# vidify/old-audiosync

Measured on AMD Instinct MI355X. Metric: cross-correlations/sec (N=1440000 float32 pairs), higher is better.
Workload: dtype f32

## Files before the change

### include/audiosync/xcorr_hip.h

```cpp
#ifndef AUDIOSYNC_XCORR_HIP_H
#define AUDIOSYNC_XCORR_HIP_H

#include <stddef.h>
#include <stdint.h>

#ifdef __cplusplus
extern "C" {
#endif

typedef struct asx_plan asx_plan;


int asx_device_count(void);
int asx_current_device(void);
const char *asx_last_error(void);
int asx_abi_version(void);


asx_plan *asx_plan_create(size_t sample_len, size_t max_batch, int device);
asx_plan *asx_plan_create_ex(size_t sample_len, size_t max_batch, int device, const char *split);
int asx_plan_placement(asx_plan *plan, double ms[2], int *kept);
void asx_plan_destroy(asx_plan *plan);

int asx_plan_peak_overflows(asx_plan *plan, uint64_t *count);
int asx_plan_peak_repairs(asx_plan *plan, uint64_t *count);
int asx_plan_set_exact(asx_plan *plan, int on);
size_t asx_plan_peak_capacity(const asx_plan *plan);

int asx_plan_set_pearson(asx_plan *plan, int spectral);
int asx_plan_pearson_modes(asx_plan *plan, uint64_t counts[3]);

size_t asx_plan_sample_len(const asx_plan *plan);
size_t asx_plan_fft_len(const asx_plan *plan);
int asx_plan_split(const asx_plan *plan, int *m1, int *m2, int *tile_cols);
int asx_plan_layout(const asx_plan *plan);
int asx_plan_threads(const asx_plan *plan, int *threads_cols, int *threads_rows);
size_t asx_plan_group(const asx_plan *plan);
size_t asx_plan_workspace_bytes(const asx_plan *plan);


int asx_xcorr_f64(asx_plan *plan, const double *source, const double *sample, long *lag,
                  double *coefficient);
int asx_plan_narrowed_calls(asx_plan *plan, uint64_t *count);

int asx_xcorr_batch_f32(asx_plan *plan, const float *source, const float *sample, size_t batch,
// ... 62 lines not shown
```

### old-audiosync_amd/csrc/asx_api.hip

```cpp
#include "audiosync/xcorr_hip.h"

#include "asx_internal.h"
#include "plan_math.h"
#include "shard_driver.h"
#include "host_narrow.h"

#include <algorithm>
#include <cstdarg>
#include <cstdio>
#include <cstdlib>
#include <cstring>
#include <dlfcn.h>
#include <mutex>
#include <string>
#include <thread>
#include <vector>

static thread_local std::string g_err;

static int fail(const char *fmt, ...)
{
    char buf[512];
    va_list ap;
    va_start(ap, fmt);
// ... 73 lines not shown
        AsxCand *cand = nullptr;
        uint32_t *refine_idx = nullptr, *cand_n = nullptr, *refine_n = nullptr;
        double *refine_val = nullptr;
        unsigned long long *overflows = nullptr;
        float *src_dc = nullptr;
        double *stats = nullptr;
        size_t cap = 0;
    } big;
    uint32_t *over_list = nullptr, *over_n = nullptr;
    volatile uint32_t *h_over_n = nullptr;
    size_t over_cap = 0;
    std::vector<uint32_t> h_over;
    unsigned long long repaired = 0;
    bool exact = true;
    bool spectral = false;
    unsigned long long *mode_count = nullptr;
    bool tune_placement = false, placement_done = false;
    double placement_ms[2] = { 0.0, 0.0 };
    int placement_kept = -1;
    float *st_src = nullptr, *st_smp = nullptr;
    int64_t *st_lag = nullptr;
    double *st_coef = nullptr;
    int32_t *st_ret = nullptr;
    double *st_src64 = nullptr, *st_smp64 = nullptr;
    float *pin32 = nullptr;
    unsigned long long narrowed = 0;

    bool profiling = false;
    size_t prof_depth = 1, prof_calls = 0, prof_ring = 0;
    std::vector<std::vector<hipEvent_t>> evr;
// ... 73 lines not shown
    cap = std::min<size_t>(cap, 2 * N);
    for (int l = 0; l < p->nlanes; l++) {
        asx_plan::Lane &ln = p->lanes[l];
        ln.pk.cap = (uint32_t)cap;
        const size_t mz = ((size_t)h.M1 + 1) * (size_t)h.M2;
        if (dev_alloc(p, &ln.zxa, g * mz) || dev_alloc(p, &ln.zya, g * mz) || dev_alloc(p, &ln.ga, g * mz) ||
            dev_alloc(p, &ln.pk.nrm_part, g * 2 * (size_t)h.ntiles) || dev_alloc(p, &ln.pk.bound2, g) ||
            dev_alloc(p, &ln.pk.pairmax, g) || dev_alloc(p, &ln.pk.cand_n, g) ||
            dev_alloc(p, &ln.pk.cand, g * cap) || dev_alloc(p, &ln.pk.refine_n, g) ||
            dev_alloc(p, &ln.pk.refine_idx, g * cap) || dev_alloc(p, &ln.pk.refine_val, g * cap) ||
            dev_alloc(p, &ln.pk.overflows, 1) ||
            dev_alloc(p, &ln.seg, g) || dev_alloc(p, &ln.psums, g * (size_t)asx_pearson_blocks((uint32_t)N) * 6))
            return -1;
        HIP_TRY(hipMemset(ln.pk.overflows, 0, sizeof(unsigned long long)));
        ln.pk.band = nullptr; ln.pk.tile_peak = nullptr;
        if (d.rlayout) {
            const size_t nbands = (size_t)d.nbands;
            if (!p->mode_count) {
                if (dev_alloc(p, &p->mode_count, ASX_PM_NMODES)) return -1;
                HIP_TRY(hipMemset(p->mode_count, 0, ASX_PM_NMODES * sizeof(unsigned long long)));
            }
            if (dev_alloc(p, &ln.pk.band, g * 2 * nbands * (size_t)h.ntiles) || dev_alloc(p, &ln.pk.tile_peak, g * (size_t)(h.M2 / h.T)) ||
                dev_alloc(p, &ln.spec.part, g * ASX_PREP_BLOCKS_MAX * 4) || dev_alloc(p, &ln.spec.hdr, g * ASX_SPEC_HDR))
                return -1;
            ln.spec.mode_count = p->mode_count;
            ln.spec.tol = 1e-5;
        }
        HIP_TRY(hipStreamCreateWithFlags(&ln.stream, hipStreamNonBlocking));
        HIP_TRY(hipEventCreateWithFlags(&ln.done, hipEventDisableTiming));
    }
    p->over_cap = std::max<size_t>(g * (size_t)p->nlanes, 1024);
    if (dev_alloc(p, &p->over_list, p->over_cap) || dev_alloc(p, &p->over_n, 1)) return -1;
    HIP_TRY(hipMemset(p->over_n, 0, sizeof(uint32_t)));
    uint32_t *d_over_host = nullptr;
    {
        void *h = nullptr, *dptr = nullptr;
        HIP_TRY(hipHostMalloc(&h, sizeof(uint32_t), hipHostMallocMapped));
        p->h_over_n = (volatile uint32_t *)h;
        *p->h_over_n = 0;
        HIP_TRY(hipHostGetDevicePointer(&dptr, h, 0));
        d_over_host = (uint32_t *)dptr;
    }
    for (int l = 0; l < p->nlanes; l++) {
        p->lanes[l].pk.over_list = p->over_list;
        p->lanes[l].pk.over_n = p->over_n;
        p->lanes[l].pk.over_host = d_over_host;
        p->lanes[l].pk.over_cap = (uint32_t)p->over_cap;
    }
    p->spectral = d.rlayout != 0;
    if (const char *e = getenv("ASX_PEARSON")) p->spectral = p->spectral && strcmp(e, "direct") != 0;
    if (const char *e = getenv("ASX_EXACT")) p->exact = atoi(e) != 0;
    HIP_TRY(hipEventCreateWithFlags(&p->fork, hipEventDisableTiming));
    d.stamps = nullptr;
    d.stamp_kernel = 0;
    if (const char *e = getenv("ASX_STAMPS")) {
        unsigned long long *st = nullptr;
        p->stamp_blocks = g * (size_t)std::max(h.M1 + 1, 2 * h.ntiles);
        if (dev_alloc(p, &st, p->stamp_blocks * 8)) return -1;
        HIP_TRY(hipMemset(st, 0, p->stamp_blocks * 8 * sizeof(unsigned long long)));
        d.stamps = st;
        d.stamp_kernel = !strcmp(e, "fwd") ? 1 : !strcmp(e, "inv") ? 2 : 0;
    }
    {
        AsxDev *dcopy = nullptr;
        if (dev_alloc(p, &dcopy, 1)) return -1;
// ... 111 lines not shown
    if (!p) return;
    int prev = 0;
    (void)hipGetDevice(&prev);
    (void)hipSetDevice(p->device);
    if (p->stream) { (void)hipStreamSynchronize(p->stream); (void)hipStreamDestroy(p->stream); }
    for (auto &ln : p->lanes) {
        if (ln.stream) { (void)hipStreamSynchronize(ln.stream); (void)hipStreamDestroy(ln.stream); }
        if (ln.done) (void)hipEventDestroy(ln.done);
    }
    if (p->fork) (void)hipEventDestroy(p->fork);
    for (auto &ring : p->evr)
        for (hipEvent_t ev : ring) (void)hipEventDestroy(ev);
    for (void *a : p->allocs) (void)hipFree(a);
    if (p->pin32) (void)hipHostFree(p->pin32);
    if (p->h_over_n) (void)hipHostFree((void *)p->h_over_n);
    (void)hipSetDevice(prev);
    delete p;
}

extern "C" size_t asx_plan_sample_len(const asx_plan *p) { return p ? p->host.N : 0; }
extern "C" size_t asx_plan_fft_len(const asx_plan *p) { return p ? p->host.F : 0; }
extern "C" size_t asx_plan_group(const asx_plan *p) { return p ? p->group : 0; }
extern "C" size_t asx_plan_workspace_bytes(const asx_plan *p) { return p ? p->ws_bytes : 0; }
extern "C" long asx_plan_debug_stamps(asx_plan *p, unsigned long long *out, size_t cap)
{
    if (!p || !p->dev.stamps) return -1;
    size_t n = p->stamp_blocks * 8;
    if (n > cap) n = cap;
    if (hipMemcpy(out, p->dev.stamps, n * sizeof(unsigned long long), hipMemcpyDeviceToHost) != hipSuccess) return -1;
    return (long)n;
// ... 27 lines not shown
    HIP_TRY(hipMemset(p->over_n, 0, sizeof(uint32_t)));
    *p->h_over_n = 0;
    p->exact = on != 0;
    return 0;
}

extern "C" int asx_plan_set_pearson(asx_plan *p, int spectral)
{
    if (!p) return fail("asx_plan_set_pearson: null argument");
    std::lock_guard<std::mutex> guard(p->lock);
    if (spectral && !p->dev.rlayout) return fail("asx_plan_set_pearson: the spectral form needs a real-column plan (the reference's six lengths)");
    p->spectral = spectral != 0;
    return 0;
}

extern "C" int asx_plan_pearson_modes(asx_plan *p, uint64_t counts[3])
{
    if (!p || !counts) return fail("asx_plan_pearson_modes: null argument");
    std::lock_guard<std::mutex> guard(p->lock);
    DevGuard dg(p->device);
    if (!dg.ok) return fail("cannot select device %d", p->device);
    counts[0] = counts[1] = counts[2] = 0;
    if (!p->mode_count) return 0;
    HIP_TRY(hipDeviceSynchronize());
    unsigned long long v[ASX_PM_NMODES];
    HIP_TRY(hipMemcpy(v, p->mode_count, sizeof v, hipMemcpyDeviceToHost));
    for (int i = 0; i < 3; i++) counts[i] = v[i];
    return 0;
}

// ... 82 lines not shown
}

template <typename TIn>
static int run_group(asx_plan *p, const float *d_src, const float *d_smp, const TIn *p_src,
                     const TIn *p_smp, size_t g, int64_t *d_lag, double *d_coef, int32_t *d_ret,
                     float *d_r, hipStream_t s, size_t group_index, int lane = 0, uint32_t pair_base = 0, bool listed = true,
                     bool float32_call = true)
{
    const AsxDev &P = p->dev;
    asx_plan::Lane &W = p->lanes[lane];
    AsxPeakWs fin = W.pk;
    if (!listed) { fin.over_list = nullptr; fin.over_n = nullptr; fin.over_host = nullptr; fin.over_cap = 0; }
    const bool spectral = p->spectral && sizeof(TIn) == sizeof(float) && float32_call && W.pk.band;
    AsxPeakWs tk = W.pk;
    if (!spectral) { tk.band = nullptr; tk.tile_peak = nullptr; }
    const size_t e0 = group_index * 6;
    if (prof_mark(p, s, e0 + 0)) return -1;
    asx_launch_fwd_cols(P, d_src, d_smp, W.zxa, W.zya, tk, (int)g, s);
    if (prof_mark(p, s, e0 + 1)) return -1;
    float2 *q = W.ga;
    asx_launch_rows(P, W.zxa, W.zya, q, tk, (int)g, s);
    if (prof_mark(p, s, e0 + 2)) return -1;
    asx_launch_inv_cols(P, q, tk, d_r, (int)g, s);
    if (prof_mark(p, s, e0 + 3)) return -1;
    asx_launch_finalize(P, fin, W.seg, (int)g, s, pair_base);
    const int dot_blocks = (int)std::min<size_t>(ASX_DOT_BLOCKS, std::max<size_t>(8, 16384 / g));
    if (sizeof(TIn) == sizeof(float))
        asx_launch_refine_f32(P, (const float *)p_src, (const float *)p_smp, W.pk, W.seg, (int)g, s, dot_blocks, !spectral);
    else
        asx_launch_refine_f64(P, (const double *)p_src, (const double *)p_smp, W.pk, W.seg, (int)g, s, dot_blocks);
    if (prof_mark(p, s, e0 + 4)) return -1;
    if (spectral)
        asx_launch_pearson_spectral_f32(P, (const float *)p_src, (const float *)p_smp, tk, W.spec, W.seg, W.psums, d_lag, d_coef,
                                        d_ret, (int)g, s);
    else if (sizeof(TIn) == sizeof(float))
        asx_launch_pearson_f32((const float *)p_src, (const float *)p_smp, 2 * (size_t)P.N, P.N, P.N,
                               W.seg, W.psums, d_lag, d_coef, d_ret, (int)g, s);
    else
// ... 16 lines not shown
        asx_plan::BigPeak T;
        T.cap = 2 * N;
        if (dev_alloc(p, &T.cand, T.cap) || dev_alloc(p, &T.refine_idx, T.cap) || dev_alloc(p, &T.refine_val, T.cap) ||
            dev_alloc(p, &T.cand_n, 1) || dev_alloc(p, &T.refine_n, 1) || dev_alloc(p, &T.overflows, 1) ||
            dev_alloc(p, &T.src_dc, 2 * N) || dev_alloc(p, &T.stats, ASX_DC_STATS_DOUBLES))
            return -1;
        HIP_TRY(hipMemsetAsync(T.overflows, 0, sizeof(unsigned long long), s));
        B = T;
    }
    AsxPeakWs K = W.pk;
    K.cand_n = B.cand_n; K.cand = B.cand;
    K.refine_n = B.refine_n; K.refine_idx = B.refine_idx; K.refine_val = B.refine_val;
    K.overflows = B.overflows;
    K.over_list = nullptr; K.over_n = nullptr; K.over_host = nullptr; K.over_cap = 0;
    K.band = nullptr; K.tile_peak = nullptr;
    K.cap = (uint32_t)B.cap;
    HIP_TRY(hipMemsetAsync(B.cand_n, 0, sizeof(uint32_t), s));
    if (sizeof(TIn) == sizeof(float))
        asx_launch_dc_remove_f32((const float *)p_src + i * 2 * N, (const float *)p_smp + i * N, P.N, (double)P.F, B.stats, B.src_dc, s);
    else
        asx_launch_dc_remove_f64((const double *)p_src + i * 2 * N, (const double *)p_smp + i * N, P.N, (double)P.F, B.stats, B.src_dc, s);
    K.shift = B.stats + 2;
    asx_launch_fwd_cols(P, B.src_dc, f_smp + i * N, W.zxa, W.zya, K, 1, s);
    asx_launch_rows(P, W.zxa, W.zya, W.ga, K, 1, s);
    asx_launch_inv_cols(P, W.ga, K, nullptr, 1, s);
    asx_launch_finalize(P, K, W.seg, 1, s);
    if (sizeof(TIn) == sizeof(float))
        asx_launch_refine_f32(P, (const float *)p_src + i * 2 * N, (const float *)p_smp + i * N, K, W.seg, 1, s, 2048);
    else
        asx_launch_refine_f64(P, (const double *)p_src + i * 2 * N, (const double *)p_smp + i * N, K, W.seg, 1, s, 2048);
    if (sizeof(TIn) == sizeof(float))
        asx_launch_pearson_f32((const float *)p_src + i * 2 * N, (const float *)p_smp + i * N, 2 * N, N, P.N,
                               W.seg, W.psums, d_lag ? d_lag + i : nullptr, d_coef + i, d_ret ? d_ret + i : nullptr, 1, s);
    else
        asx_launch_pearson_f64((const double *)p_src + i * 2 * N, (const double *)p_smp + i * N, 2 * N, N, P.N,
                               W.seg, W.psums, d_lag ? d_lag + i : nullptr, d_coef + i, d_ret ? d_ret + i : nullptr, 1, s);
    HIP_TRY(hipGetLastError());
    p->repaired++;
    return 0;
}

template <typename TIn>
static int resolve_overflows(asx_plan *p, const float *f_smp, const TIn *p_src, const TIn *p_smp, int64_t *d_lag,
                             double *d_coef, int32_t *d_ret, hipStream_t s)
{
    HIP_TRY(hipStreamSynchronize(s));
    if (p->lanes[0].pk.cap >= 2 * p->host.N) return 0;
    const uint32_t n = *p->h_over_n;
    if (n == 0) return 0;
    if (n > p->over_cap) {
        (void)hipMemsetAsync(p->over_n, 0, sizeof(uint32_t), s);
        (void)hipStreamSynchronize(s);
        *p->h_over_n = 0;
        return fail("internal: %u overflowed pairs in a window of %zu", n, p->over_cap);
    }
    p->h_over.resize(n);
    HIP_TRY(hipMemcpyAsync(p->h_over.data(), p->over_list, n * sizeof(uint32_t), hipMemcpyDeviceToHost, s));
    HIP_TRY(hipMemsetAsync(p->over_n, 0, sizeof(uint32_t), s));
    HIP_TRY(hipStreamSynchronize(s));
    *p->h_over_n = 0;
    for (uint32_t k = 0; k < n; k++)
// ... 845 lines not shown
```

### old-audiosync_amd/csrc/asx_internal.h

```cpp
#pragma once

#include <hip/hip_runtime.h>
#include <stdint.h>

#define ASX_MAX_STAGES 12
#define ASX_TW_LOG 11
#define ASX_TW_LO (1u << ASX_TW_LOG)
#define ASX_THREADS 256
#define ASX_FFT_THREADS_MAX 512
#define ASX_COL_LOADS 10
#define ASX_ROW_STEPS 5
#define ASX_PEARSON_BLOCKS_MAX 512
#define ASX_DC_STATS_DOUBLES (4 + 2 * 128)
#define ASX_BOUND_C 4.0f
#define ASX_CAND_MAX 16384
#define ASX_CAND_MIN 2048
#define ASX_DOT_BLOCKS 128

struct AsxStages {
    int n;
    int nstages;
    int radix[ASX_MAX_STAGES];
    int ns[ASX_MAX_STAGES];
    int q[ASX_MAX_STAGES];
// ... 57 lines not shown
    asx_peak_t *pairmax;
    uint32_t *cand_n;
    AsxCand *cand;
    uint32_t *refine_n;
    uint32_t *refine_idx;
    double *refine_val;
    unsigned long long *overflows;
    uint32_t *over_list;
    uint32_t *over_n;
    uint32_t *over_host;
    uint32_t over_cap;
    const double *shift;
    uint32_t cap;
    float2 *band;
    float *tile_peak;
};

#define ASX_PM_FAST 0
#define ASX_PM_CORR 1
#define ASX_PM_DIRECT 2
#define ASX_PM_NMODES 3
#ifndef ASX_PREP_BLOCKS
#define ASX_PREP_BLOCKS 4
#endif
#define ASX_PREP_BLOCKS_MAX 16
#define ASX_SPEC_HDR 4
struct AsxSpecWs {
    double *part;
    double *hdr;
    unsigned long long *mode_count;
// ... 2 lines not shown
    uint32_t N;
};

void asx_launch_fwd_cols(const AsxDev &P, const float *src, const float *smp, float2 *zxa,
                         float2 *zya, const AsxPeakWs &W, int npairs, hipStream_t s);
void asx_launch_rows(const AsxDev &P, const float2 *zxa, const float2 *zya, float2 *ga,
                     const AsxPeakWs &W, int npairs, hipStream_t s);
void asx_launch_inv_cols(const AsxDev &P, const float2 *ga, const AsxPeakWs &W, float *r_out,
                         int npairs, hipStream_t s);
bool asx_launch_rows_r(const AsxDev &P, const float2 *cx, const float2 *cy, float2 *q, const AsxPeakWs &W, int npairs,
                       hipStream_t s);
bool asx_launch_fwd_cols_r(const AsxDev &P, const float *src, const float *smp, float2 *cx, float2 *cy, const AsxPeakWs &W,
                           int npairs, hipStream_t s);
bool asx_launch_inv_cols_r(const AsxDev &P, const float2 *q, const AsxPeakWs &W, float *r_out, int npairs, hipStream_t s);
bool asx_rlayout_available(const AsxDev &P);
int asx_rlayout_band_rows(const AsxDev &P);
void asx_launch_finalize(const AsxDev &P, const AsxPeakWs &W, AsxSeg *seg, int npairs, hipStream_t s, uint32_t pair_base = 0);
void asx_launch_refine_f32(const AsxDev &P, const float *src, const float *smp, const AsxPeakWs &W,
                           AsxSeg *seg, int npairs, hipStream_t s, int dot_blocks = ASX_DOT_BLOCKS, bool pick = true);
void asx_launch_refine_f64(const AsxDev &P, const double *src, const double *smp, const AsxPeakWs &W,
                           AsxSeg *seg, int npairs, hipStream_t s, int dot_blocks = ASX_DOT_BLOCKS);
void asx_launch_pearson_f32(const float *src, const float *smp, size_t src_pitch, size_t smp_pitch,
                            uint32_t basis_len, const AsxSeg *seg, double *psums, int64_t *lag,
                            double *coef, int32_t *ret, int npairs, hipStream_t s);
void asx_launch_pearson_f64(const double *src, const double *smp, size_t src_pitch, size_t smp_pitch,
                            uint32_t basis_len, const AsxSeg *seg, double *psums, int64_t *lag,
                            double *coef, int32_t *ret, int npairs, hipStream_t s);
void asx_launch_pearson_partial_spec_f32(const float *src, const float *smp, size_t src_pitch, size_t smp_pitch, uint32_t basis_len,
                                         const AsxSeg *seg, const AsxSpecWs &S, double *psums, int npairs, hipStream_t s);
void asx_launch_pearson_spectral_f32(const AsxDev &P, const float *src, const float *smp, const AsxPeakWs &W, const AsxSpecWs &S,
// ... 15 lines not shown
```

### old-audiosync_amd/csrc/rlayout.hip

```cpp
#include "asx_internal.h"
#include "lds_fft.h"
#include "xcorr_dev.h"

#include <initializer_list>
#include <map>
#include <mutex>
#include <utility>
#include <stdlib.h>

extern __shared__ __attribute__((aligned(16))) float2 asx_lds_r[];

#ifdef ASX_STAMPS
#define RSTAMP(kernel, block, slot)                                                                  \
    do {                                                                                             \
        if (P.stamps && P.stamp_kernel == (kernel) && threadIdx.x == 0)                              \
            P.stamps[(size_t)(block) * 8 + (slot)] = clock64();                                      \
    } while (0)
#else
#define RSTAMP(kernel, block, slot) do {} while (0)
#endif

struct RArgs {
    const float2 *tw1, *tw2, *tw_lo, *tw_hi;
    uint32_t N, nout;
// ... 11 lines not shown
    return a;
}
__device__ __forceinline__ float2 tw_F(const RArgs &P, uint32_t p)
{
    const float2 lo = P.tw_lo[p & (ASX_TW_LO - 1u)];
    const float2 hi = P.tw_hi[p >> ASX_TW_LOG];
    return cmul(lo, hi);
}

__device__ __forceinline__ Cx1 lds_get1(const float4 *p)
{
    const float2 x = *reinterpret_cast<const float2 *>(p);
    return Cx1{ x.x, x.y };
}
__device__ __forceinline__ void lds_put1(float4 *p, Cx1 v) { *reinterpret_cast<float2 *>(p) = make_float2(v.re, v.im); }

__device__ __forceinline__ void wave_lds_sync()
{
    asm volatile("s_waitcnt lgkmcnt(0)" ::: "memory");
    __builtin_amdgcn_fence(__ATOMIC_RELEASE, "wavefront");
    __builtin_amdgcn_wave_barrier();
    __builtin_amdgcn_fence(__ATOMIC_ACQUIRE, "wavefront");
}

__device__ __forceinline__ float quad_sum(float v)
{
    v += __int_as_float(__builtin_amdgcn_mov_dpp(__float_as_int(v), 0xB1, 0xF, 0xF, true));
    v += __int_as_float(__builtin_amdgcn_mov_dpp(__float_as_int(v), 0x4E, 0xF, 0xF, true));
    return v;
}
// ... 238 lines not shown
    if constexpr (!TWO) {
        for (int j = lt; j < Q0; j += NT) {
            const float4 *p = A4 + j;
            Cx1 v[R0];
            static_for<0, R0>([&](auto T) __attribute__((always_inline)) { v[T] = lds_get1(p + decltype(T)::value * Q0); });
            float2 w1 = s0w1, w4 = s0w4, fb = tw0base;
            if (j != lt) { w1 = P.tw2[j]; w4 = P.tw2[4 * j]; fb = tw_F(P, k1 * (uint32_t)j); }
            float2 tww[R0];
            stage_twiddles_from<R0>(w1, w4, tww);
            static_for<1, R0>([&](auto U) __attribute__((always_inline)) { v[U] = mulwc(v[U], tww[U]); });
            Bfly<R0, true>::run(v);
            static_for<0, R0>([&](auto T) __attribute__((always_inline)) {
                constexpr int t = decltype(T)::value;
                const Cx1 y = mulwc(v[t], t == 0 ? fb : cmul(fb, leg[t]));
                st_f2(go + j + t * Q0, make_float2(y.re, y.im), ASX_RNT & 8);
            });
        }
    } else {
        const float4 *base = reinterpret_cast<const float4 *>(asx_lds_r);
        static_assert(Q0 <= NT, "one butterfly per thread of the first half");
        for (int j = tid; j < Q0; j += NTB) {
            Cx2 v[R0];
            static_for<0, R0>([&](auto T) __attribute__((always_inline)) {
                const Cx1 a = lds_get1(base + j + decltype(T)::value * Q0), b = lds_get1(base + NS + j + decltype(T)::value * Q0);
                v[T] = Cx2{ v2f{ a.re, b.re }, v2f{ a.im, b.im } };
            });
            float2 tww[R0];
            if constexpr (ASX_ROWS_EARLY & 2) stage_twiddles_from<R0>(s0w1, s0w4, tww);
            else stage_twiddles_from<R0>(P.tw2[TWS * j], P.tw2[TWS * 4 * j], tww);
            static_for<1, R0>([&](auto U) __attribute__((always_inline)) { v[U] = mulwc(v[U], tww[U]); });
            Bfly<R0, true>::run(v);
            const float2 w2 = (ASX_ROWS_EARLY & 2) ? tail_w2 : P.tw2[j];
            const float2 fa = (ASX_ROWS_EARLY & 2) ? cmul(tail_lo, tail_hi) : tw_F(P, k1 * (uint32_t)j);
            const float2 fbh = cmul(fa, wh);
            static_for<0, R0>([&](auto T) __attribute__((always_inline)) {
                constexpr int t = decltype(T)::value;
                const Cx1 A = Cx1{ v[t].re.x, v[t].im.x };
                const Cx1 Bw = mul_root<2 * R0, t, true>(mulwc(Cx1{ v[t].re.y, v[t].im.y }, w2));
                const float2 lg = leg[t];
                const Cx1 y = mulwc(A + Bw, t == 0 ? fa : cmul(fa, lg));
                const Cx1 z = mulwc(A - Bw, t == 0 ? fbh : cmul(fbh, lg));
                st_f2(go + j + t * Q0, make_float2(y.re, y.im), ASX_RNT & 8);
                st_f2(go + NS + j + t * Q0, make_float2(z.re, z.im), ASX_RNT & 8);
            });
        }
    }
    RSTAMP(0, task, 4);
#ifdef ASX_STAMPS
    if (P.stamps && P.stamp_kernel == 0 && threadIdx.x == 0) P.stamps[(size_t)task * 8 + 5] = wall_clock64();
#endif
}

__device__ __host__ constexpr int rcol_line_log(int logT) { return logT >= 5 ? 0 : 5 - logT; }
__device__ __forceinline__ int rcol_tile_of_block(int b, int logT)
{
    const int ll = rcol_line_log(logT);
    const int grp = 8 << ll;
    return (b & ~(grp - 1)) + ((b & 7) << ll) + ((b >> 3) & ((1 << ll) - 1));
}
// ... 129 lines not shown
                if constexpr (t == 0) row(M1, S - wd, true);
            });
            static_for<0, RL>([&](auto TT) __attribute__((always_inline)) {
                constexpr int t = decltype(TT)::value;
                const Cx2 a = zb[t], bq = zb[RL - 1 - t];
                const Cx2 S = Cx2{ a.re + bq.re, a.im - bq.im };
                const Cx2 Dm = Cx2{ a.im + bq.im, bq.re - a.re };
                const Cx2 wd = mul_root<4 * RL, 2 * t + 1, false>(Dm);
                row(MB / 2 + MB * t, S + wd, false);
            });
        }
    }
}

template <class S1, int TC, int NT>
__global__ __launch_bounds__(NT, 4) void k_inv_cols_r(const RArgs P, const float2 *__restrict__ qi, size_t pair_pitch,
                                                       AsxPeakWs W, float *__restrict__ r_out, unsigned first_gen)
{
    constexpr int M1 = S1::n, T = TC, logT = asx_ilog2(TC), H = T / 2, logH = logT - 1;
    __shared__ asx_peak_t red[NT / 64];
    __shared__ asx_peak_t s_run0;
    __shared__ float s_b2;
    const size_t pair = blockIdx.x;
    const int tile = rcol_tile_of_block(blockIdx.y, logT);
    if (tile * T >= P.M2) return;
    {
        const unsigned lin = blockIdx.x + gridDim.x * blockIdx.y;
        if (gridDim.x * gridDim.y > first_gen && lin < first_gen && (lin & 1u))
            for (unsigned i = 0; i < (unsigned)(M1 * 27 / 64 / 2); i += 16) __builtin_amdgcn_s_sleep(16);
    }
    const double shift = W.shift ? W.shift[pair] : 0.0;
    const int M2 = P.M2, c0 = tile * T;
    const float2 *in = qi + RWS_PAIR(pair) * pair_pitch;
    float4 *lds4 = reinterpret_cast<float4 *>(asx_lds_r);
    const LdsLayout Lc = col_layout(T, logT, NT);
    const float b2_early = W.bound2[pair];
    asx_peak_t run0_early = 0;
    if (threadIdx.x == 0) run0_early = W.pairmax[pair];
    static_assert(S1::nstages == 3, "three-stage column schedules");
    constexpr StageK KL = S1::stage(2), KM = S1::stage(1);
    constexpr int RL = KL.R, R0c = S1::stage(0).R, R1c = KM.R, MB = M1 / RL;
    static_assert(KL.q == 1 && MB == R0c * R1c && MB % 2 == 0, "innermost stage of consecutive slots");
    constexpr int NITEMS = (MB / 2) * H;
// ... 151 lines not shown
            });
        });
        const asx_peak_t mine = best_idx == 0xFFFFFFFFu ? 0 : peak_pack_key(best_key, best_idx);
        asx_peak_t best = block_peak_max(mine, red);
        if (threadIdx.x == 0) { atomicMax(&W.pairmax[pair], best); red[0] = best; }
        __syncthreads();
        if (W.tile_peak && mine != 0 && mine == red[0]) W.tile_peak[pair * (size_t)(P.M2 / T) + tile] = best_val;
        const float thr = near_max_threshold(peak_key(peak_max(red[0], run0)), b2);
        again = best_key >= thr;
        thr_again = thr;
    }
    if (again) examine_again(thr_again);
    RSTAMP(2, sblock, 3);
}

static bool schedule_is_r(const AsxStages &st, int n, std::initializer_list<int> radices)
{
    if (st.n != n || st.nstages != (int)radices.size()) return false;
    int i = 0;
    for (int r : radices)
        if (st.radix[i++] != r) return false;
    return true;
}

bool asx_launch_rows_r(const AsxDev &P, const float2 *cx, const float2 *cy, float2 *q, const AsxPeakWs &W, int npairs,
                       hipStream_t s)
{
    const int nrows = P.M1 + 1;
    const size_t pitch = (size_t)nrows * (size_t)P.M2;
    const size_t lds = (size_t)P.M2 * sizeof(float4);
// ... 46 lines not shown
    if (P.T == (t) && schedule_is_r(P.st1, m1, { __VA_ARGS__ })) {                                    \
        allow_big_lds_r((const void *)k_fwd_cols_r<Sched<m1, __VA_ARGS__>, t, nt>, lds);                                    \
        hipLaunchKernelGGL((k_fwd_cols_r<Sched<m1, __VA_ARGS__>, t, nt>), grid, dim3(nt), lds, s, rargs_of(P), src, smp, cx, cy, \
                           W.nrm_part, pitch, W.band);                                                                      \
        return true;                                                                                                        \
    }
    ASX_RCOLS(ASX_TRY)
#undef ASX_TRY
    return false;
}

bool asx_launch_inv_cols_r(const AsxDev &P, const float2 *q, const AsxPeakWs &W, float *r_out, int npairs, hipStream_t s)
{
    if (!P.col_pairs) return false;
    const size_t pitch = ((size_t)P.M1 + 1) * (size_t)P.M2;
#define ASX_TRY(m1, t, nt, ...)                                                                                             \
    if (P.T == (t) && schedule_is_r(P.st1, m1, { __VA_ARGS__ })) {                               \
        const size_t lds = (size_t)(m1) * (t) * sizeof(float2);                                                             \
        const dim3 grid(npairs, rcol_grid_x(P.M2 / (t), asx_ilog2(t)));                                                     \
        const void *fn = (const void *)k_inv_cols_r<Sched<m1, __VA_ARGS__>, t, nt>;                                         \
        allow_big_lds_r(fn, lds);                                                                                           \
        hipLaunchKernelGGL((k_inv_cols_r<Sched<m1, __VA_ARGS__>, t, nt>), grid, dim3(nt), lds, s, rargs_of(P), q, pitch, W, r_out, \
                           resident_blocks(fn, nt, lds));                                                                   \
        return true;                                                                                                        \
    }
    ASX_RCOLS(ASX_TRY)
#undef ASX_TRY
    return false;
}

int asx_rlayout_band_rows(const AsxDev &P)
{
#define ASX_TRY(m1, t, nt, ...) if (P.T == (t) && schedule_is_r(P.st1, m1, { __VA_ARGS__ })) return 2 * rcol_rows_per_group(m1, nt, t);
    ASX_RCOLS(ASX_TRY)
#undef ASX_TRY
    return 0;
}

bool asx_rlayout_available(const AsxDev &P)
// ... 10 lines not shown
```

### old-audiosync_amd/hipxcorr.py

```python
import ctypes
import os
import sys

import numpy as np

_HERE = os.path.dirname(os.path.abspath(__file__))
LIB_PATH = os.path.join(_HERE, "libaudiosync_hip.so")
_lib = None

c_f32p = ctypes.POINTER(ctypes.c_float)
c_f64p = ctypes.POINTER(ctypes.c_double)
c_i64p = ctypes.POINTER(ctypes.c_int64)
c_i32p = ctypes.POINTER(ctypes.c_int32)
c_intp = ctypes.POINTER(ctypes.c_int)

ABI_SYMBOLS = [
    "asx_device_count", "asx_last_error", "asx_abi_version", "asx_plan_create", "asx_plan_create_ex", "asx_plan_destroy",
    "asx_plan_sample_len", "asx_plan_fft_len", "asx_plan_split", "asx_plan_threads", "asx_plan_group",
    "asx_plan_workspace_bytes", "asx_xcorr_f64", "asx_xcorr_batch_f32", "asx_xcorr_batch_f32_dev",
    "asx_xcorr_debug_r_dev", "asx_pearson_f64", "asx_results_to_ms_dev", "asx_stream_create", "asx_stream_destroy",
    "asx_stream_append_f64", "asx_stream_lengths", "asx_stream_reset", "asx_stream_xcorr", "asx_synth_pairs_dev", "asx_plan_set_profiling",
    "asx_plan_last_timings_ms", "asx_device_malloc", "asx_device_free", "asx_memcpy_h2d",
    "asx_memcpy_d2h", "asx_stream_sync", "asx_plan_peak_overflows", "asx_plan_peak_repairs", "asx_plan_set_exact", "asx_plan_peak_capacity",
    "asx_current_device", "asx_plan_timings_ms", "asx_xcorr_batch_multi", "asx_plan_layout", "asx_plan_narrowed_calls",
    "asx_plan_set_pearson", "asx_plan_pearson_modes", "asx_plan_placement", "asx_host_malloc", "asx_host_free", "asx_shard_range", "asx_result_bytes", "asx_comm_create", "asx_comm_destroy", "asx_xcorr_batch_multi_dev",
]


class AsxError(RuntimeError):
    pass


def _one_hip_runtime():
    if os.environ.get("ASX_NO_TORCH") == "1" or "torch" in sys.modules:
        return
    try:
        import torch
    except ImportError:
        pass

# ... 15 lines not shown
    L.asx_plan_create.argtypes = [ctypes.c_size_t, ctypes.c_size_t, ctypes.c_int]
    L.asx_plan_create_ex.restype = vp
    L.asx_plan_create_ex.argtypes = [ctypes.c_size_t, ctypes.c_size_t, ctypes.c_int, ctypes.c_char_p]
    L.asx_plan_destroy.restype = None
    L.asx_plan_destroy.argtypes = [vp]
    L.asx_plan_peak_overflows.restype = ctypes.c_int
    L.asx_plan_peak_overflows.argtypes = [vp, ctypes.POINTER(ctypes.c_uint64)]
    L.asx_plan_set_exact.restype = ctypes.c_int
    L.asx_plan_set_exact.argtypes = [vp, ctypes.c_int]
    L.asx_plan_placement.restype = ctypes.c_int
    L.asx_plan_placement.argtypes = [vp, ctypes.POINTER(ctypes.c_double), ctypes.POINTER(ctypes.c_int)]
    L.asx_plan_set_pearson.restype = ctypes.c_int
    L.asx_plan_set_pearson.argtypes = [vp, ctypes.c_int]
    L.asx_plan_pearson_modes.restype = ctypes.c_int
    L.asx_plan_pearson_modes.argtypes = [vp, ctypes.POINTER(ctypes.c_uint64)]
    L.asx_plan_peak_repairs.restype = ctypes.c_int
    L.asx_plan_peak_repairs.argtypes = [vp, ctypes.POINTER(ctypes.c_uint64)]
    L.asx_plan_narrowed_calls.restype = ctypes.c_int
    L.asx_plan_narrowed_calls.argtypes = [vp, ctypes.POINTER(ctypes.c_uint64)]
    for name in ("asx_plan_sample_len", "asx_plan_fft_len", "asx_plan_group", "asx_plan_workspace_bytes",
                 "asx_plan_peak_capacity"):
        getattr(L, name).restype = ctypes.c_size_t
        getattr(L, name).argtypes = [vp]
    L.asx_plan_threads.restype = ctypes.c_int
    L.asx_plan_threads.argtypes = [vp, c_intp, c_intp]
    L.asx_plan_split.restype = ctypes.c_int
    L.asx_plan_split.argtypes = [vp, c_intp, c_intp, c_intp]
    L.asx_plan_layout.restype = ctypes.c_int
    L.asx_plan_layout.argtypes = [vp]
    L.asx_xcorr_f64.restype = ctypes.c_int
# ... 318 lines not shown
        kept = ctypes.c_int(-1)
        if lib().asx_plan_placement(self._h, ms, ctypes.byref(kept)) != 0:
            raise AsxError(_err())
        return (float(ms[0]), float(ms[1])), int(kept.value)

    def set_pearson(self, spectral=True):
        if lib().asx_plan_set_pearson(self._h, 1 if spectral else 0) != 0:
            raise AsxError(_err())

    def pearson_modes(self):
        c = (ctypes.c_uint64 * 3)()
        if lib().asx_plan_pearson_modes(self._h, c) != 0:
            raise AsxError(_err())
        return tuple(int(v) for v in c)

    def narrowed_calls(self):
        c = ctypes.c_uint64(0)
        if lib().asx_plan_narrowed_calls(self._h, ctypes.byref(c)) != 0:
            raise AsxError(_err())
        return c.value

    def peak_repairs(self):
        c = ctypes.c_uint64(0)
        if lib().asx_plan_peak_repairs(self._h, ctypes.byref(c)) != 0:
            raise AsxError(_err())
        return c.value

    @property
    def workspace_bytes(self):
        return lib().asx_plan_workspace_bytes(self._h)
# ... 69 lines not shown
```

Before: 54930.

## Prune inverse column tiles using per-tile energy bounds on the correlation peak

The row stage now records per-row, per-16-column-tile spectral energy. A new kernel reduces this energy into a Cauchy-Schwarz-style upper bound on each tile's correlation magnitude. The inverse-column pass then runs in two phases: first the tile with the highest bound establishes a running peak, then any other tile whose bound falls below the near-max threshold is skipped. A host-side feedback loop turns pruning off for a while when most tiles still run, which adds bound computation, extra launches, LDS energy writes and an async counter copy as overhead.

```diff
diff --git a/include/audiosync/xcorr_hip.h b/include/audiosync/xcorr_hip.h
--- a/include/audiosync/xcorr_hip.h
+++ b/include/audiosync/xcorr_hip.h
@@ -29,6 +29,10 @@
 
 int asx_plan_set_pearson(asx_plan *plan, int spectral);
 int asx_plan_pearson_modes(asx_plan *plan, uint64_t counts[3]);
+
+int asx_plan_set_prune(asx_plan *plan, int on);
+int asx_plan_prune_stats(asx_plan *plan, uint64_t *tiles_total, uint64_t *tiles_transformed);
+long asx_plan_debug_tile_bounds(asx_plan *plan, float *out, size_t cap);
 
 size_t asx_plan_sample_len(const asx_plan *plan);
 size_t asx_plan_fft_len(const asx_plan *plan);
diff --git a/old-audiosync_amd/csrc/asx_api.hip b/old-audiosync_amd/csrc/asx_api.hip
--- a/old-audiosync_amd/csrc/asx_api.hip
+++ b/old-audiosync_amd/csrc/asx_api.hip
@@ -111,6 +111,11 @@
     unsigned long long repaired = 0;
     bool exact = true;
     bool spectral = false;
+    bool prune = true;
+    unsigned long long tiles_total = 0, tiles_unpruned = 0;
+    unsigned long long *h_tiles_run = nullptr;
+    unsigned long long pruned_tiles = 0, look_run = 0, look_tiles = 0;
+    int prune_skip = 0;
     unsigned long long *mode_count = nullptr;
     bool tune_placement = false, placement_done = false;
     double placement_ms[2] = { 0.0, 0.0 };
@@ -214,6 +219,7 @@
             return -1;
         HIP_TRY(hipMemset(ln.pk.overflows, 0, sizeof(unsigned long long)));
         ln.pk.band = nullptr; ln.pk.tile_peak = nullptr;
+        ln.pk.energy = nullptr; ln.pk.tbound = nullptr; ln.pk.ttop = nullptr; ln.pk.tiles_run = nullptr;
         if (d.rlayout) {
             const size_t nbands = (size_t)d.nbands;
             if (!p->mode_count) {
@@ -225,6 +231,11 @@
                 return -1;
             ln.spec.mode_count = p->mode_count;
             ln.spec.tol = 1e-5;
+            const size_t et = (size_t)(h.M2 / 16);
+            if (dev_alloc(p, &ln.pk.energy, g * ((size_t)h.M1 + 1) * et) || dev_alloc(p, &ln.pk.tbound, g * et) ||
+                dev_alloc(p, &ln.pk.ttop, g) || dev_alloc(p, &ln.pk.tiles_run, 1))
+                return -1;
+            HIP_TRY(hipMemset(ln.pk.tiles_run, 0, sizeof(unsigned long long)));
         }
         HIP_TRY(hipStreamCreateWithFlags(&ln.stream, hipStreamNonBlocking));
         HIP_TRY(hipEventCreateWithFlags(&ln.done, hipEventDisableTiming));
@@ -238,6 +249,10 @@
         HIP_TRY(hipHostMalloc(&h, sizeof(uint32_t), hipHostMallocMapped));
         p->h_over_n = (volatile uint32_t *)h;
         *p->h_over_n = 0;
+        void *t = nullptr;
+        HIP_TRY(hipHostMalloc(&t, 2 * sizeof(unsigned long long), hipHostMallocDefault));
+        p->h_tiles_run = (unsigned long long *)t;
+        p->h_tiles_run[0] = p->h_tiles_run[1] = 0;
         HIP_TRY(hipHostGetDevicePointer(&dptr, h, 0));
         d_over_host = (uint32_t *)dptr;
     }
@@ -249,6 +264,7 @@
     }
     p->spectral = d.rlayout != 0;
     if (const char *e = getenv("ASX_PEARSON")) p->spectral = p->spectral && strcmp(e, "direct") != 0;
+    if (const char *e = getenv("ASX_PRUNE")) p->prune = atoi(e) != 0;
     if (const char *e = getenv("ASX_EXACT")) p->exact = atoi(e) != 0;
     HIP_TRY(hipEventCreateWithFlags(&p->fork, hipEventDisableTiming));
     d.stamps = nullptr;
@@ -390,6 +406,7 @@
     for (void *a : p->allocs) (void)hipFree(a);
     if (p->pin32) (void)hipHostFree(p->pin32);
     if (p->h_over_n) (void)hipHostFree((void *)p->h_over_n);
+    if (p->h_tiles_run) (void)hipHostFree(p->h_tiles_run);
     (void)hipSetDevice(prev);
     delete p;
 }
@@ -447,6 +464,48 @@
     return 0;
 }
 
+extern "C" int asx_plan_set_prune(asx_plan *p, int on)
+{
+    if (!p) return fail("asx_plan_set_prune: null argument");
+    std::lock_guard<std::mutex> guard(p->lock);
+    p->prune = on != 0;
+    p->prune_skip = 0;
+    return 0;
+}
+
+extern "C" long asx_plan_debug_tile_bounds(asx_plan *p, float *out, size_t cap)
+{
+    if (!p || !out) return fail("asx_plan_debug_tile_bounds: null argument");
+    std::lock_guard<std::mutex> guard(p->lock);
+    if (!p->lanes[0].pk.tbound) return fail("asx_plan_debug_tile_bounds: the plan does not prune (not a real-column plan)");
+    DevGuard dg(p->device);
+    if (!dg.ok) return fail("cannot select device %d", p->device);
+    size_t n = p->group * (size_t)(p->host.M2 / 16);
+    if (n > cap) n = cap;
+    HIP_TRY(hipDeviceSynchronize());
+    HIP_TRY(hipMemcpy(out, p->lanes[0].pk.tbound, n * sizeof(float), hipMemcpyDeviceToHost));
+    return (long)n;
+}
+
+extern "C" int asx_plan_prune_stats(asx_plan *p, uint64_t *tiles_total, uint64_t *tiles_transformed)
+{
+    if (!p || !tiles_total || !tiles_transformed) return fail("asx_plan_prune_stats: null argument");
+    std::lock_guard<std::mutex> guard(p->lock);
+    DevGuard dg(p->device);
+    if (!dg.ok) return fail("cannot select device %d", p->device);
+    unsigned long long run = 0;
+    for (int l = 0; l < p->nlanes; l++) {
+        unsigned long long v = 0;
+        HIP_TRY(hipStreamSynchronize(p->lanes[l].stream));
+        HIP_TRY(hipStreamSynchronize(p->stream));
+        if (p->lanes[l].pk.tiles_run) HIP_TRY(hipMemcpy(&v, p->lanes[l].pk.tiles_run, sizeof(v), hipMemcpyDeviceToHost));
+        run += v;
+    }
+    *tiles_total = p->tiles_total;
+    *tiles_transformed = p->tiles_unpruned + run;
+    return 0;
+}
+
 extern "C" int asx_plan_pearson_modes(asx_plan *p, uint64_t counts[3])
 {
     if (!p || !counts) return fail("asx_plan_pearson_modes: null argument");
@@ -559,6 +618,14 @@
     const bool spectral = p->spectral && sizeof(TIn) == sizeof(float) && float32_call && W.pk.band;
     AsxPeakWs tk = W.pk;
     if (!spectral) { tk.band = nullptr; tk.tile_peak = nullptr; }
+    bool prune = p->prune && P.rlayout && !d_r && W.pk.energy && asx_rlayout_prune_pays(P, (int)g);
+    if (prune && p->prune_skip > 0) { p->prune_skip--; prune = false; }
+    if (prune) p->pruned_tiles += g * (size_t)(P.M2 / P.T);
+    if (!prune) { tk.energy = nullptr; tk.tbound = nullptr; tk.ttop = nullptr; tk.tiles_run = nullptr; }
+    if (P.rlayout) {
+        p->tiles_total += g * (size_t)(P.M2 / P.T);
+        if (!prune) p->tiles_unpruned += g * (size_t)(P.M2 / P.T);
+    }
     const size_t e0 = group_index * 6;
     if (prof_mark(p, s, e0 + 0)) return -1;
     asx_launch_fwd_cols(P, d_src, d_smp, W.zxa, W.zya, tk, (int)g, s);
@@ -567,6 +634,8 @@
     asx_launch_rows(P, W.zxa, W.zya, q, tk, (int)g, s);
     if (prof_mark(p, s, e0 + 2)) return -1;
     asx_launch_inv_cols(P, q, tk, d_r, (int)g, s);
+    if (prune && p->h_tiles_run)
+        HIP_TRY(hipMemcpyAsync(p->h_tiles_run + lane, tk.tiles_run, sizeof(unsigned long long), hipMemcpyDeviceToHost, s));
     if (prof_mark(p, s, e0 + 3)) return -1;
     asx_launch_finalize(P, fin, W.seg, (int)g, s, pair_base);
     const int dot_blocks = (int)std::min<size_t>(ASX_DOT_BLOCKS, std::max<size_t>(8, 16384 / g));
@@ -613,6 +682,7 @@
     K.overflows = B.overflows;
     K.over_list = nullptr; K.over_n = nullptr; K.over_host = nullptr; K.over_cap = 0;
     K.band = nullptr; K.tile_peak = nullptr;
+    K.energy = nullptr; K.tbound = nullptr; K.ttop = nullptr; K.tiles_run = nullptr;
     K.cap = (uint32_t)B.cap;
     HIP_TRY(hipMemsetAsync(B.cand_n, 0, sizeof(uint32_t), s));
     if (sizeof(TIn) == sizeof(float))
@@ -639,11 +709,25 @@
     return 0;
 }
 
+#ifndef ASX_PRUNE_BACKOFF
+#define ASX_PRUNE_BACKOFF 16
+#endif
+static void prune_look(asx_plan *p)
+{
+    if (!p->h_tiles_run) return;
+    const unsigned long long run = p->h_tiles_run[0] + p->h_tiles_run[1];
+    const unsigned long long dr = run - p->look_run, dt = p->pruned_tiles - p->look_tiles;
+    p->look_run = run;
+    p->look_tiles = p->pruned_tiles;
+    if (dt > 0 && 2 * dr > dt) p->prune_skip = ASX_PRUNE_BACKOFF;
+}
+
 template <typename TIn>
 static int resolve_overflows(asx_plan *p, const float *f_smp, const TIn *p_src, const TIn *p_smp, int64_t *d_lag,
                              double *d_coef, int32_t *d_ret, hipStream_t s)
 {
     HIP_TRY(hipStreamSynchronize(s));
+    prune_look(p);
     if (p->lanes[0].pk.cap >= 2 * p->host.N) return 0;
     const uint32_t n = *p->h_over_n;
     if (n == 0) return 0;
diff --git a/old-audiosync_amd/csrc/asx_internal.h b/old-audiosync_amd/csrc/asx_internal.h
--- a/old-audiosync_amd/csrc/asx_internal.h
+++ b/old-audiosync_amd/csrc/asx_internal.h
@@ -95,6 +95,10 @@
     uint32_t cap;
     float2 *band;
     float *tile_peak;
+    float *energy;
+    float *tbound;
+    int *ttop;
+    unsigned long long *tiles_run;
 };
 
 #define ASX_PM_FAST 0
@@ -127,6 +131,7 @@
                            int npairs, hipStream_t s);
 bool asx_launch_inv_cols_r(const AsxDev &P, const float2 *q, const AsxPeakWs &W, float *r_out, int npairs, hipStream_t s);
 bool asx_rlayout_available(const AsxDev &P);
+bool asx_rlayout_prune_pays(const AsxDev &P, int npairs);
 int asx_rlayout_band_rows(const AsxDev &P);
 void asx_launch_finalize(const AsxDev &P, const AsxPeakWs &W, AsxSeg *seg, int npairs, hipStream_t s, uint32_t pair_base = 0);
 void asx_launch_refine_f32(const AsxDev &P, const float *src, const float *smp, const AsxPeakWs &W,
diff --git a/old-audiosync_amd/csrc/rlayout.hip b/old-audiosync_amd/csrc/rlayout.hip
--- a/old-audiosync_amd/csrc/rlayout.hip
+++ b/old-audiosync_amd/csrc/rlayout.hip
@@ -49,6 +49,8 @@
     return Cx1{ x.x, x.y };
 }
 __device__ __forceinline__ void lds_put1(float4 *p, Cx1 v) { *reinterpret_cast<float2 *>(p) = make_float2(v.re, v.im); }
+__device__ __forceinline__ void put_energy(float4 *p, Cx1 v) { reinterpret_cast<float2 *>(p)[1] = make_float2(v.re, v.im); }
+#define ASX_ETILE 16
 
 __device__ __forceinline__ void wave_lds_sync()
 {
@@ -317,6 +319,7 @@
                 constexpr int t = decltype(T)::value;
                 const Cx1 y = mulwc(v[t], t == 0 ? fb : cmul(fb, leg[t]));
                 st_f2(go + j + t * Q0, make_float2(y.re, y.im), ASX_RNT & 8);
+                if (W.energy) put_energy(A4 + j + t * Q0, y);
             });
         }
     } else {
@@ -345,7 +348,23 @@
                 const Cx1 z = mulwc(A - Bw, t == 0 ? fbh : cmul(fbh, lg));
                 st_f2(go + j + t * Q0, make_float2(y.re, y.im), ASX_RNT & 8);
                 st_f2(go + NS + j + t * Q0, make_float2(z.re, z.im), ASX_RNT & 8);
-            });
+                put_energy(reinterpret_cast<float4 *>(asx_lds_r) + j + t * Q0, y);
+                put_energy(reinterpret_cast<float4 *>(asx_lds_r) + NS + j + t * Q0, z);
+            });
+        }
+    }
+    if (W.energy) {
+        static_assert(M2 % ASX_ETILE == 0 && NTB % ASX_ETILE == 0 && ASX_ETILE == 16, "whole tiles, one DPP row each");
+        __syncthreads();
+        const float4 *e4 = reinterpret_cast<const float4 *>(asx_lds_r);
+        float *eo = W.energy + ((size_t)pair * nrows + k1) * (M2 / ASX_ETILE);
+        for (int c = tid; c < M2; c += NTB) {
+            const float2 q = reinterpret_cast<const float2 *>(e4 + c)[1];
+            float e = fmaf(q.x, q.x, q.y * q.y);
+            e = quad_sum(e);
+            e += __int_as_float(__builtin_amdgcn_mov_dpp(__float_as_int(e), 0x124, 0xF, 0xF, false));
+            e += __int_as_float(__builtin_amdgcn_mov_dpp(__float_as_int(e), 0x128, 0xF, 0xF, false));
+            if ((c & (ASX_ETILE - 1)) == 0) eo[c / ASX_ETILE] = e;
         }
     }
     RSTAMP(0, task, 4);
@@ -505,19 +524,16 @@
 }
 
 template <class S1, int TC, int NT>
-__global__ __launch_bounds__(NT, 4) void k_inv_cols_r(const RArgs P, const float2 *__restrict__ qi, size_t pair_pitch,
-                                                       AsxPeakWs W, float *__restrict__ r_out, unsigned first_gen)
+__device__ __forceinline__ void inv_cols_r_tile(const RArgs &P, const float2 *__restrict__ qi, size_t pair_pitch, const AsxPeakWs &W,
+                                                float *__restrict__ r_out, const size_t pair, const int tile, const bool stagger)
 {
     constexpr int M1 = S1::n, T = TC, logT = asx_ilog2(TC), H = T / 2, logH = logT - 1;
     __shared__ asx_peak_t red[NT / 64];
     __shared__ asx_peak_t s_run0;
     __shared__ float s_b2;
-    const size_t pair = blockIdx.x;
-    const int tile = rcol_tile_of_block(blockIdx.y, logT);
     if (tile * T >= P.M2) return;
     {
-        const unsigned lin = blockIdx.x + gridDim.x * blockIdx.y;
-        if (gridDim.x * gridDim.y > first_gen && lin < first_gen && (lin & 1u))
+        if (stagger)
             for (unsigned i = 0; i < (unsigned)(M1 * 27 / 64 / 2); i += 16) __builtin_amdgcn_s_sleep(16);
     }
     const double shift = W.shift ? W.shift[pair] : 0.0;
@@ -699,6 +715,83 @@
     RSTAMP(2, sblock, 3);
 }
 
+template <class S1, int TC, int NT>
+__global__ __launch_bounds__(NT, 4) void k_inv_cols_r(const RArgs P, const float2 *__restrict__ qi, size_t pair_pitch,
+                                                       AsxPeakWs W, float *__restrict__ r_out, unsigned first_gen)
+{
+    const unsigned lin = blockIdx.x + gridDim.x * blockIdx.y;
+    const bool stagger = gridDim.x * gridDim.y > first_gen && lin < first_gen && (lin & 1u);
+    inv_cols_r_tile<S1, TC, NT>(P, qi, pair_pitch, W, r_out, blockIdx.x, rcol_tile_of_block(blockIdx.y, asx_ilog2(TC)), stagger);
+}
+
+
+__global__ __launch_bounds__(256) void k_tile_bounds(const float *__restrict__ energy, float *__restrict__ tbound, int nrows, int ntiles,
+                                                     double scale)
+{
+    __shared__ double part[16][17];
+    const int tl = threadIdx.x & 15, sl = threadIdx.x >> 4, tile = blockIdx.y * 16 + tl;
+    const size_t pair = blockIdx.x;
+    double s = 0.0;
+    if (tile < ntiles) {
+        const float *e = energy + pair * (size_t)nrows * ntiles + tile;
+#pragma unroll 8
+        for (int k = sl; k < nrows; k += 16) s += (double)e[(size_t)k * ntiles];
+    }
+    part[sl][tl] = s;
+    __syncthreads();
+    if (threadIdx.x < 16 && tile < ntiles) {
+        double t = 0.0;
+        for (int i = 0; i < 16; i++) t += part[i][tl];
+        const double b = sqrt(scale * t) * (1.0 + 1e-3);
+        float f = (float)b;
+        if ((double)f < b) f = nextafterf(f, INFINITY);
+        tbound[pair * ntiles + tile] = f;
+    }
+}
+
+template <class S1, int TC, int NT>
+__global__ __launch_bounds__(NT, 4) void k_inv_cols_rp(const RArgs P, const float2 *__restrict__ qi, size_t pair_pitch, AsxPeakWs W,
+                                                        unsigned first_gen, int phase)
+{
+    static_assert(TC == ASX_ETILE, "the bounds are per tile of this width");
+    const int ntiles = P.M2 / TC;
+    const size_t pair = blockIdx.x;
+    int tile = 0;
+    bool stagger = false;
+    if (phase == 0) {
+        if (blockIdx.y != 0) {
+            __shared__ asx_peak_t s_red[NT / 64];
+            __shared__ int s_top;
+            const float *b = W.tbound + pair * (size_t)ntiles;
+            asx_peak_t mine = 0;
+            for (int t = threadIdx.x; t < ntiles; t += NT) {
+                const float v = b[t];
+                if (v >= 0.f) {
+                    const asx_peak_t k = ((asx_peak_t)__float_as_uint(v) << 32) | (asx_peak_t)(0xFFFFFFFFu - (uint32_t)t);
+                    mine = k > mine ? k : mine;
+                }
+            }
+            const asx_peak_t best = block_peak_max(mine, s_red);
+            if (threadIdx.x == 0) {
+                s_top = best ? (int)(0xFFFFFFFFu - (uint32_t)best) : 0;
+                W.ttop[pair] = s_top;
+            }
+            __syncthreads();
+            tile = __builtin_amdgcn_readfirstlane(s_top);
+            if (tile == 0) return;
+        }
+    } else {
+        tile = rcol_tile_of_block(blockIdx.y, asx_ilog2(TC));
+        if (tile == 0 || tile >= ntiles) return;
+        const float thr = near_max_threshold(peak_key(W.pairmax[pair]), W.bound2[pair]);
+        if (W.ttop[pair] == tile || W.tbound[pair * (size_t)ntiles + tile] < thr) return;
+        const unsigned lin = blockIdx.x + gridDim.x * blockIdx.y;
+        stagger = gridDim.x * gridDim.y > first_gen && lin < first_gen && (lin & 1u);
+    }
+    if (threadIdx.x == 0) atomicAdd(W.tiles_run, 1ull);
+    inv_cols_r_tile<S1, TC, NT>(P, qi, pair_pitch, W, nullptr, pair, tile, stagger);
+}
+
 static bool schedule_is_r(const AsxStages &st, int n, std::initializer_list<int> radices)
 {
     if (st.n != n || st.nstages != (int)radices.size()) return false;
@@ -775,15 +868,43 @@
 {
     if (!P.col_pairs) return false;
     const size_t pitch = ((size_t)P.M1 + 1) * (size_t)P.M2;
+    const bool prune = W.energy && W.tbound && W.ttop && W.tiles_run && !r_out && !W.shift && P.T == ASX_ETILE;
 #define ASX_TRY(m1, t, nt, ...)                                                                                             \
     if (P.T == (t) && schedule_is_r(P.st1, m1, { __VA_ARGS__ })) {                               \
         const size_t lds = (size_t)(m1) * (t) * sizeof(float2);                                                             \
+        if (prune) {                                                                                                        \
+            const int nt16 = P.M2 / ASX_ETILE;                                                                              \
+            hipLaunchKernelGGL(k_tile_bounds, dim3(npairs, (nt16 + 15) / 16), dim3(256), 0, s, W.energy, W.tbound, P.M1 + 1, \
+                               nt16, 4.0 * (double)P.M1);                                                                   \
+            const void *fp = (const void *)k_inv_cols_rp<Sched<m1, __VA_ARGS__>, t, nt>;                                    \
+            allow_big_lds_r(fp, lds);                                                                                       \
+            const unsigned fg = resident_blocks(fp, nt, lds);                                                              \
+            hipLaunchKernelGGL((k_inv_cols_rp<Sched<m1, __VA_ARGS__>, t, nt>), dim3(npairs, 2), dim3(nt), lds, s, rargs_of(P), \
+                               q, pitch, W, fg, 0);                                                                         \
+            hipLaunchKernelGGL((k_inv_cols_rp<Sched<m1, __VA_ARGS__>, t, nt>), dim3(npairs, rcol_grid_x(P.M2 / (t), asx_ilog2(t))), \
+                               dim3(nt), lds, s, rargs_of(P), q, pitch, W, fg, 1);                                          \
+            return true;                                                                                                    \
+        }                                                                                                                   \
         const dim3 grid(npairs, rcol_grid_x(P.M2 / (t), asx_ilog2(t)));                                                     \
         const void *fn = (const void *)k_inv_cols_r<Sched<m1, __VA_ARGS__>, t, nt>;                                         \
         allow_big_lds_r(fn, lds);                                                                                           \
         hipLaunchKernelGGL((k_inv_cols_r<Sched<m1, __VA_ARGS__>, t, nt>), grid, dim3(nt), lds, s, rargs_of(P), q, pitch, W, r_out, \
                            resident_blocks(fn, nt, lds));                                                                   \
         return true;                                                                                                        \
+    }
+    ASX_RCOLS(ASX_TRY)
+#undef ASX_TRY
+    return false;
+}
+
+bool asx_rlayout_prune_pays(const AsxDev &P, int npairs)
+{
+    if (!P.col_pairs || P.T != ASX_ETILE) return false;
+#define ASX_TRY(m1, t, nt, ...)                                                                                             \
+    if (P.T == (t) && schedule_is_r(P.st1, m1, { __VA_ARGS__ })) {                                                          \
+        allow_big_lds_r((const void *)k_inv_cols_r<Sched<m1, __VA_ARGS__>, t, nt>, (size_t)(m1) * (t) * sizeof(float2));    \
+        return (size_t)npairs * (size_t)(P.M2 / (t)) >                                                                      \
+               resident_blocks((const void *)k_inv_cols_r<Sched<m1, __VA_ARGS__>, t, nt>, nt, (size_t)(m1) * (t) * sizeof(float2)); \
     }
     ASX_RCOLS(ASX_TRY)
 #undef ASX_TRY
diff --git a/old-audiosync_amd/hipxcorr.py b/old-audiosync_amd/hipxcorr.py
--- a/old-audiosync_amd/hipxcorr.py
+++ b/old-audiosync_amd/hipxcorr.py
@@ -24,6 +24,7 @@
     "asx_memcpy_d2h", "asx_stream_sync", "asx_plan_peak_overflows", "asx_plan_peak_repairs", "asx_plan_set_exact", "asx_plan_peak_capacity",
     "asx_current_device", "asx_plan_timings_ms", "asx_xcorr_batch_multi", "asx_plan_layout", "asx_plan_narrowed_calls",
     "asx_plan_set_pearson", "asx_plan_pearson_modes", "asx_plan_placement", "asx_host_malloc", "asx_host_free", "asx_shard_range", "asx_result_bytes", "asx_comm_create", "asx_comm_destroy", "asx_xcorr_batch_multi_dev",
+    "asx_plan_set_prune", "asx_plan_prune_stats", "asx_plan_debug_tile_bounds",
 ]
 
 
@@ -69,6 +70,12 @@
     L.asx_plan_set_pearson.argtypes = [vp, ctypes.c_int]
     L.asx_plan_pearson_modes.restype = ctypes.c_int
     L.asx_plan_pearson_modes.argtypes = [vp, ctypes.POINTER(ctypes.c_uint64)]
+    L.asx_plan_set_prune.restype = ctypes.c_int
+    L.asx_plan_set_prune.argtypes = [vp, ctypes.c_int]
+    L.asx_plan_prune_stats.restype = ctypes.c_int
+    L.asx_plan_prune_stats.argtypes = [vp, ctypes.POINTER(ctypes.c_uint64), ctypes.POINTER(ctypes.c_uint64)]
+    L.asx_plan_debug_tile_bounds.restype = ctypes.c_long
+    L.asx_plan_debug_tile_bounds.argtypes = [vp, c_f32p, ctypes.c_size_t]
     L.asx_plan_peak_repairs.restype = ctypes.c_int
     L.asx_plan_peak_repairs.argtypes = [vp, ctypes.POINTER(ctypes.c_uint64)]
     L.asx_plan_narrowed_calls.restype = ctypes.c_int
@@ -417,6 +424,24 @@
             raise AsxError(_err())
         return tuple(int(v) for v in c)
 
+    def set_prune(self, on=True):
+        if lib().asx_plan_set_prune(self._h, 1 if on else 0) != 0:
+            raise AsxError(_err())
+
+    def prune_stats(self):
+        t, r = ctypes.c_uint64(0), ctypes.c_uint64(0)
+        if lib().asx_plan_prune_stats(self._h, ctypes.byref(t), ctypes.byref(r)) != 0:
+            raise AsxError(_err())
+        return int(t.value), int(r.value)
+
+    def debug_tile_bounds(self):
+        m1, m2, t = self.split
+        out = np.zeros(self.group * (m2 // 16), dtype=np.float32)
+        n = lib().asx_plan_debug_tile_bounds(self._h, out.ctypes.data_as(c_f32p), out.size)
+        if n < 0:
+            raise AsxError(_err())
+        return out.reshape(self.group, m2 // 16)
+
     def narrowed_calls(self):
         c = ctypes.c_uint64(0)
         if lib().asx_plan_narrowed_calls(self._h, ctypes.byref(c)) != 0:
```

New measurement: 59490, median of 6. 8.3% higher.
